# adelacvg/detail_tts

Hardware: AMD Instinct MI355X
Metric: generated audio seconds/sec (24 kHz), 10 s prompt, batch 8 per GPU (higher is better)
Workload: dtype f32; 1 GPU; configs[2]: 1xMI355X batch-8, 10 s prompts (T_ref=936), 234 codes -> 9.984 s audio per utterance; GPT KV-cache decode + 50-step CFG diffusion + flow-VAE/HiFiGAN vocoder, seed-0 random-init weights; batch_per_gpu=8, codes=234, diffusion_steps=50, parallelism=replica x1

## Files before the change

detail_tts_amd/csrc/conv_x3.hip:

```cpp
#include <algorithm>
#include <atomic>
#include <cstdio>
#include <mutex>
#include <type_traits>
#include <utility>
#include <vector>

#include "conv_x3.h"
#include <cstdlib>
#include "prof.h"
#include "split3.h"

namespace dtts {

typedef float f32x16 __attribute__((ext_vector_type(16)));

namespace {
constexpr int NPL = XS_PLANES, NK = 2 * NPL;
constexpr int BM = 128, BN = X3_BN;
constexpr int WTILE = NK * BM * 16;
constexpr int XMAIN = NK * BN * 16;
constexpr int XBUF = XMAIN + NK * 2 * 16;

__global__ __launch_bounds__(256) void split_weights_kernel(const float* __restrict__ wp, int C8, int CoutP, uint4* __restrict__ out) {
// ... 875 lines not shown
    static const long long split_wgs = env_int("DTTS_CONV_KSPLIT_WGS", 256);
    const long long ntile_pad = (long long)(CoutP / BM) * cdiv(Nout, BN) * B;
    static const int max_split_k1 = env_int("DTTS_CONV_KSPLIT_K1", 2);
    if (ntile_pad <= split_tiles) S = (int)std::min<long long>(std::min<long long>(KW == 3 ? max_split : std::min(max_split, max_split_k1), split_wgs / ntile_pad), (Cin >> 4) / 8);
    if (ksplit_max > 0) S = std::min(S, ksplit_max);
    return S < 1 ? 1 : S;
}

static int conv_stages_default() {
    static const int v = []() { const int n = (int)env_int("DTTS_CONV_STAGES", 0); return n >= 2 && n <= 4 ? n : 0; }();
    return v;
}
static std::atomic<int> g_conv_stages{-1};
void set_conv_stages(int n) {
    DTTS_REQUIRE(n <= 0 || (n >= 2 && n <= 4), "conv_stages: 0 (by launch size), 2, 3 or 4");
    g_conv_stages.store(n < 0 ? -1 : n, std::memory_order_relaxed);
}

void launch_conv_x3(const ConvParams& p_in, hipStream_t s, ConvX3Launch* chosen) {
    ConvParams p = p_in;
    DTTS_REQUIRE(p.w3 && p.x3 && (p.y || p.qkv_planes) && p.x3_tp > 0, "conv_x3: operands");
    static const int env_ablate = env_int("DTTS_CONV_ABLATE", 0);
    if (env_ablate) p.ablate = env_ablate;
    DTTS_REQUIRE(p.B > 0 && p.Nout > 0 && p.Cout > 0, "empty conv");
    DTTS_REQUIRE(p.Cin % 16 == 0 && p.CoutP % BM == 0, "conv_x3: channel padding");
    const bool p1 = p.p1 != 0;
    DTTS_REQUIRE(!p1 || (p.Cin % 32 == 0 && p.gate == GATE_NONE), "conv_x3 one-product mode: input channels a multiple of 32, no gate");
    const bool gated = p.gate == GATE_TANH_SIGMOID;
    DTTS_REQUIRE(p.stride == 1 && p.dil == 1 && p.phases == 1 && (p.gate == GATE_NONE ? !p.badd : gated), "conv_x3: unsupported conv form");
    DTTS_REQUIRE(!gated || (p.KW == 1 && !p.qkv_planes && !p.res && p.epi_act == ACT_NONE && p.out_scale == 1.f && p.Cout % 2 == 0),
                 "conv_x3 gated epilogue: 1x1 conv, no residual / activation");
    DTTS_REQUIRE((p.KW == 1 && p.pad == 0) || (p.KW == 3 && p.pad == 1), "conv_x3: k = 1 or k = 3 (same padding) only");
    DTTS_REQUIRE(round_up(p.Nout, BN) + 2 * X3_HALO <= p.x3_tp, "conv_x3: time padding");
    const int stg_opt = g_conv_stages.load(std::memory_order_relaxed);
    const int force_stg = stg_opt >= 0 ? stg_opt : conv_stages_default();
    static const long long max3 = env_int("DTTS_CONV_STAGES3_MAXWG", 600);
    static const long long max4 = env_int("DTTS_CONV_STAGES4_MAXWG", 128);
    DTTS_REQUIRE(!p.cols || (p.ncols > 0 && p.ncols <= cdiv(p.Nout, BN) * p.B && cdiv(p.Nout, BN) < 256), "conv_x3: column table");
    const long long ntile = (long long)(p.CoutP / BM) * (p.cols ? p.ncols : cdiv(p.Nout, BN) * p.B);
    const int S = conv_x3_ksplit(p.CoutP, p.Cin, p.KW, p.Nout, p.B, p.ksplit_max);
    p.ksplit = S;
    static const bool epi_vec_on = env_on("DTTS_X3_EPI_VEC");
    auto al16 = [](const void* q, long long bs, int cs) { return (reinterpret_cast<unsigned long long>(q) & 15ull) == 0 && (bs & 3) == 0 && (cs & 3) == 0; };
    p.epi_vec = (epi_vec_on && p.y && al16(p.y, p.y_bs, p.y_cs) && (!p.res || al16(p.res, p.res_bs, p.res_cs))) ? 1 : 0;
    if (S > 1) {
        const KSplitWs w = ksplit_workspace(s, (size_t)ntile * S);
        p.kpart = w.part;
        p.kcount = w.count;
    }
    const long long nwg = ntile * S;
    static const long long max4k3 = env_int("DTTS_CONV_STAGES4_MAXWG_K3", 128);
    const int nstg = force_stg ? force_stg : (nwg <= (p.KW == 3 ? max4k3 : max4) ? 4 : (nwg <= max3 ? 3 : 2));
    const size_t lds = (size_t)nstg * (WTILE + XBUF) + BM * sizeof(float) + 16;
    const int l4 = 4 * (WTILE + XBUF) + BM * (int)sizeof(float) + 16;
    const dim3 grid((unsigned)nwg);
    const double cols = (double)p.B * p.Nout;
    const double flops = 2.0 * p.Cout * p.Cin * p.KW * cols;
    const double bytes = 4.0 * cols * p.Cin + 4.0 * cols * p.Cout * (p.res ? 2.0 : 1.0) + 4.0 * (double)p.Cout * p.Cin * p.KW;
    {
        static const bool by_shape = []() { const char* v = env_str("DTTS_PROF_SHAPES"); return v && v[0] == '1'; }();
        const char* tag = p1 ? "conv_x3_kernel<128,192,fp16>" : "conv_x3_kernel<128,192>";
        if (by_shape && p1) tag = p.KW == 3 ? "conv_x3 fp16 k3" : (p.Cout > 1024 ? "conv_x3 fp16 k1 M=2304" : (p.res ? "conv_x3 fp16 k1 +res" : "conv_x3 fp16 k1"));
        else if (by_shape) tag = p.KW == 3 ? "conv_x3 k3" : (p.Cout > 1024 ? "conv_x3 k1 M=2304" : (p.res ? "conv_x3 k1 +res" : "conv_x3 k1"));
        ProfScope ps(tag, flops, bytes, s);
        const bool epi = p.epi_act != ACT_NONE || p.out_scale != 1.f;
        if (chosen) {
// ... 48 lines not shown
```

detail_tts_amd/csrc/model.h:

```cpp
#pragma once
#include <map>
#include <memory>
#include <atomic>
#include <thread>
#include <cstring>
#include <memory>
#include <mutex>
#include <string>
#include <unordered_map>
#include <vector>

#include "attention.h"
#include "attn_probs.h"
#include "common.h"
#include "conv_gemm.h"
#include "conv_x3.h"
#include "diff_loss.h"
#include "diff_schedule.h"
#include "disc.h"
#include "flowvae_fwd.h"
#include "gpt_kernels.h"
#include "ops.h"
#include "uncond_cache.h"
#include "../../include/detail_hip.h"

namespace dtts {

struct PackedConv {
    const float* w = nullptr;
    const float* b = nullptr;
    int Cin = 0, CinP = 0, Cout = 0, CoutP = 0, KW = 1;
    const void* w3 = nullptr;
};

static inline int packed_cout(int cout) { return cout > 64 ? round_up(cout, 128) : (cout > 32 ? 64 : 32); }

static inline int gn_groups(int C) {
    int groups = 32;
    while (C % groups) groups /= 2;
    return groups;
}

struct AttnBlockW {
    const float *gn_g = nullptr, *gn_b = nullptr, *bias_tab = nullptr;
    PackedConv qkv, proj;
    int C = 0, H = 0;
};

struct ResBlockW {
    const float *gn1_g = nullptr, *gn1_b = nullptr, *gn2_g = nullptr, *gn2_b = nullptr;
    PackedConv c1, c2, emb;
    int index = 0;
};

struct DiffLayerW {
// ... 305 lines not shown
    void op_attention_x3(const char* name, const float* x, const int* lens_host, int B, int Cin, int T, int H, const float* bias_tab, int p1,
                         int out_f32, void* y, void* img_out, ConvX3Launch* conv_chosen, AttnX3Launch* attn_chosen, hipStream_t s);
    void op_attention(const float* qkv, const int* lens_host, int B, int rows, int cs, int T, int H, int D, int q_off, int k_off, int v_off,
                      int head_stride, float scale, const float* bias_tab, int causal, const float* band, int band_w, float* y, float* ml,
                      hipStream_t s);
    void op_attention_rel(const float* qkv, const int* lens_host, int B, int T, int H, int D, const float* ek, const float* ev, int W,
                          float scale, float* y, float* relk, float* ml, hipStream_t s);
    void op_philox_normal(float* out, int n, int B, unsigned long long seed, const int* sample_ids_host, int stage, int step,
                          hipStream_t s);

    void set_option(const std::string& key, int value) {
        if (key == "two_streams") opt_two_streams_ = value != 0;
        else if (key == "conv_x3") {
            DTTS_REQUIRE(value != 0 || !opt_trunk_fp16_, "conv_x3 = 0 (exact fp32 kernels) has no trunk_fp16 mode: set trunk_fp16 = 0 first");
            opt_conv_x3_ = value != 0;
        }
        else if (key == "trunk_fp16") {
            DTTS_REQUIRE(value == 0 || value == 1, "trunk_fp16: 0 or 1");
            DTTS_REQUIRE(value == 0 || use_x3(), "trunk_fp16 = 1 needs the split-precision kernels (conv_x3 = 1): the exact fp32 kernels have no one-product mode");
            opt_trunk_fp16_ = value != 0;
        }
        else if (key == "gpt_graph") opt_gpt_graph_ = value != 0;
        else if (key == "x3_range_check") opt_range_check_ = value != 0;
        else if (key == "gpt_token_kernel") { opt_gpt_token_ = value != 0; if (value != 0) tok_failed_ = false; gpt_drop_graphs(); }
        else if (key == "gpt_fuse_proj") { DTTS_REQUIRE(value == 0 || value == 1, "gpt_fuse_proj: 0 or 1"); opt_gpt_fuse_proj_ = value != 0; gpt_drop_graphs(); }
        else if (key == "gpt_token_exclusive_cu") { opt_tok_exclusive_ = value != 0; gpt_drop_graphs(); }
        else if (key == "gpt_token_min_rows") { DTTS_REQUIRE(value == 1 || value == 4 || value == 8, "gpt_token_min_rows: 1, 4 or 8"); opt_tok_min_rows_ = value; gpt_drop_graphs(); }
        else if (key == "gpt_token_wgs") { DTTS_REQUIRE(value == 128 || value == 64 || value == 32, "gpt_token_wgs: 128, 64 or 32"); opt_tok_wgs_ = value; gpt_drop_graphs(); }
        else if (key == "gpt_token_fault") opt_tok_fault_ = value;
        else if (key == "gpt_token_fault_eos") opt_tok_fault_eos_ = value;
        else if (key == "gpt_prompt_raw") opt_prompt_raw_ = value != 0;
        else if (key == "gpt_beam_skip_reorder") { opt_beam_skip_reorder_ = value != 0; gpt_drop_graphs(); }
        else if (key == "cfg_streams") opt_cfg_streams_ = value < 0 ? 0 : value;
        else if (key == "conv_cols") opt_conv_cols_ = value != 0;
        else if (key == "uncond_cache_mb") set_uncond_cache_mb(value);
        else if (key == "voc_chain_planes") opt_voc_chain_ = value != 0;
        else if (key == "voc_x3") opt_voc_x3_ = value != 0;
        else if (key == "x3_fault") opt_x3_fault_ = value;
        else if (key == "attn_ksplit_cus") set_attn_ksplit_cus(value);
        else if (key == "attn_ksplit") set_attn_ksplit(value);
        else if (key == "ln_reg") set_ln_channels_reg(value != 0);
        else if (key == "conv_small_tiles") set_conv_small_tiles(value);
        else if (key == "conv_stages") set_conv_stages(value);
        else throw Error(-1, "unknown option '" + key + "'");
    }
    int get_option(const std::string& key) const {
        if (key == "conv_x3") return use_x3() ? 1 : 0;
        if (key == "trunk_fp16") return opt_trunk_fp16_ ? 1 : 0;
        if (key == "gpt_fuse_proj") return opt_gpt_fuse_proj_ ? 1 : 0;
        throw Error(-1, "option '" + key + "' cannot be read back");
    }
    std::string last_error;
    dtts_config cfg;
    int device;

private:
    friend struct Stage;
    const float* W(const std::string& name, size_t numel) const;
    const float* Wopt(const std::string& name, size_t numel) const;
    PackedConv conv(const std::string& name, int Cin, int Cout, int KW, bool bias = true, int cout_p = 0) const;
    AttnBlockW attn_block(const std::string& prefix, int C, int H) const;
    ResBlockW res_block(const std::string& prefix, int C, int index) const;
    void resblock1_fwd(const ResBlock1W& rb, const float* x, float* tmp, float* out, int ch, const int* lens, int B, int T, hipStream_t s,
                       void* xs = nullptr);
    bool vocoder_x3() const;
    void wn_fwd(const WnW& c, float* h, const float* g, int gin, float* Gc, float* acts, float* h2, float* skip, const int* dl, int B,
// ... 37 lines not shown
    void build_vq();
    void build_frontend();
    void gpt_prefill_layers(float* x, const int* lens, int B, int L, float* kv_cache, long long kv_layer_stride, long long kv_bs,
                            int kv_cs, hipStream_t s, const GptAttnCapture* capture = nullptr);
    void gpt_capture_probs(const GptAttnCapture& c, int layer, const float* qkv, const int* lens, int B, int L, hipStream_t s);
    MelStyleW mel_style_w(const std::string& prefix, int n_mel, int hidden, int out) const;
    ConvParams cp(const float* x, int cin, float* y, int cout, int B, int T, int Ta, const int* lens) const;
    ConvParams cp(const float* x, int cin, int Tin, int Tin_a, const int* len_in, float* y, int cout, int Nout, int Nout_a, const int* len_out,
                  int B) const;
    static void with_planes(ConvParams& p, const void* xs, int T) { p.x3 = xs; p.x3_tp = x3_tp(T); }
    static void with_res(ConvParams& p, const float* res, long long bs, int cs) { p.res = res; p.res_bs = bs; p.res_cs = cs; }

    const int* upload_ints(const int* host, int n, hipStream_t s);
    void register_cols(const int* lens_dev, const int* lens_host, int nb, int T, hipStream_t s);

    void run_conv(const PackedConv& pc, ConvParams p, hipStream_t s, ConvX3Launch* chosen = nullptr) const;
    struct TrunkIo {
        const int* lens;
        int B, T, Ta;
        hipStream_t s;
        float* ab;
        void* xs = nullptr;
        bool p1 = false;
        const int* step_idx = nullptr;
    };
    void norm_input(const float* x, int C, const float* gamma, const float* beta, int act, bool x3, const TrunkIo& io);
    void attention_block(const AttnBlockW& w, const float* x, float* y, float* qkv, float* att, const TrunkIo& io);
    void res_block_fwd(const Schedule& sc, const ResBlockW& w, const float* x, float* h1, float* y, int step, const TrunkIo& io);
    void res_block_front(const ResBlockW& w, const float* x, float* h1, const TrunkIo& io);
    void res_block_back(const Schedule& sc, const ResBlockW& w, const float* h1, const float* x, float* y, int step, const TrunkIo& io, int bmod = 0,
                        const int* bidx = nullptr);
    void code_half(const float* in, float* P, const TrunkIo& io);
    bool use_x3() const;
    struct PairPlan { const int *lens2, *lens_i, *umap, *xmap; int Nu; std::vector<int> lens_i_host; };
    PairPlan plan_pair(const int* lens_host, int B, int T, hipStream_t s);
    void diff_forward_pair(const Schedule& sc, const float* x, const float* cbuf0, const PairPlan& pl, int B, int T, int step, float* out2,
                           hipStream_t s, const float* integ = nullptr, const int* umap = nullptr);
    void precompute_integrator(const Schedule& sc, const float* cbuf0, const int* lens_i, const int* lens_i_host, int B, int Nu, int T,
                               const std::vector<int>& steps, float* integ_all, hipStream_t s, int J = 0);
    struct PairCall { PairPlan pl; const int* sids; float *cbuf0, *out2, *hist; bool uncond_deferred; };
    PairCall begin_pair(const float* code_emb, const int* lens_host, const int* sample_ids_host, int B, int T, hipStream_t s,
                        size_t extra_bytes = 0, size_t hist_floats = 0, bool defer_uncond = false);
    void draw_x_T(float* x, const PairCall& pc, const int* lens_host, int B, int T, unsigned long long seed, hipStream_t s);
    struct CodePathTable {
        float* base = nullptr;
        int k0 = 0;
        size_t stride = 0;
        const int* umap = nullptr;
        int umap_stride = 0;
        const float* at(int k) const { return base ? base + (size_t)(k - k0) * stride : nullptr; }
        const int* umap_at(int k) const { return umap ? umap + (size_t)(k - k0) * umap_stride : nullptr; }
    };
    CodePathTable code_path_table(const Schedule& sc, const PairCall& pc, int B, int T, int k_first, int k_end, bool descending, bool pinned,
                                  hipStream_t s);
    enum { SAMPLER_DDIM_REVERSE = 3 };
    void sampler_update(const Schedule& sc, const PairCall& pc, float* x, int B, int T, int sampler, float eta, int step,
                        unsigned long long seed, int pstep, const float* noise, int denorm, hipStream_t s, float* x0_out = nullptr,
                        float* x0_hist = nullptr);
    struct SampleLoop {
        int sampler = 0;
        float eta = 0.f;
        int k_first = 0, k_end = 0;
        int resample = 1;
        const float* known = nullptr;
        const unsigned char* keep = nullptr;
        const float *known_noise = nullptr, *renoise = nullptr;
        const float* step_noise = nullptr;
        float* x_traj = nullptr;
        int denorm = 0;
    };
    void sample_loop(Schedule& sc, const SampleLoop& c, const float* code_emb, const int* lens_host, int B, int T, unsigned long long seed,
                     const int* sample_ids_host, const float* x_init, float* x, hipStream_t s);
    template <class Update>
    void single_step(Schedule& sc, const float* x, const float* code_emb, const int* lens_host, const int* sample_ids_host, int B, int T,
                     int step, bool pinned_table, hipStream_t s, Update&& update);
    void ensure_fork_events();
    void diff_forward_rows_s(const Schedule& sc, const float* x, const float* code_emb, const int* lens_host, int B, int T, const int* step_of_row,
                             float* out, hipStream_t s);
    size_t rows_ws_bytes(int B, int C, int T) const;
    const Schedule& loss_schedule(int sched_id, const int* t_host, int B, const char* who);
    const DiffLossCoefs* upload_loss_coefs(const Schedule& sc, const int* t_host, int B, hipStream_t s);

    std::unordered_map<std::string, std::pair<const float*, size_t>> weights_;
    bool bound_ = false;

    std::vector<DiffLayerW> integ_, layers_;
    std::vector<ResBlockW> tail_;
    std::vector<AttnBlockW> latcond_, ctx_;
    PackedConv xpath_;
    PackedConv integ2_, out_conv_, latcond0_, ctx0_, ctx1_, te0_, te2_;
    const float *out_gn_g_ = nullptr, *out_gn_b_ = nullptr, *code_gn_g_ = nullptr, *code_gn_b_ = nullptr, *uncond_ = nullptr;
    int n_resblocks_ = 0;
    Schedule sched0_;
    static constexpr size_t MAX_SCHEDULES = 8;
    std::vector<std::unique_ptr<Schedule>> sched_cache_;
    int sched_next_id_ = 1;
    std::mutex sched_mu_;
    Schedule& schedule(int id);
    void diff_forward_s(Schedule& sc, const float* x, const float* code_emb, const int* lens_host, int B, int T, int step, int cond_free,
                        float* out, hipStream_t s);
    void build_ss_table(const Schedule& sc, float* ss_table, float* scratch, void* ts_dev, hipStream_t s);
    int cache_schedule(std::unique_ptr<Schedule> key, hipStream_t s);

    MelStyleW ref_enc_, gpt_cond_;
    bool has_vocoder_ = false, has_gpt_ = false;
    PackedConv in_proj_, enc_out_, enc_proj_, dec_pre_, dec_cond_, dec_post_;
    std::vector<EncLayerW> enc_layers_;
    std::vector<CouplingW> flows_;
    PosteriorW enc_q_;
    bool has_enc_q_ = false;
    std::vector<GenStageW> gen_;

// ... 63 lines not shown
    bool ucache_slot_busy(int slot);
    bool integ_unsplit(int Bi_lo, int Bi_hi, int T, int n_pos, int J) const;
public:
    UncondCacheStats uncond_cache_stats();
private:
    int prof_rot_ = 0;
    bool opt_voc_x3_ = true;
    int opt_x3_fault_ = 0;
    bool opt_voc_chain_ = true;
    bool opt_conv_cols_ = true;
    bool opt_range_check_ = false;
    static constexpr int X3_SAT_SLOTS = 8;
    int* x3_sat_ = nullptr;
    int* x3_sat_ring_dev_ = nullptr;
    int* x3_sat_dev_ = nullptr;
    long long x3_ticket_ = 0;
    int* x3_sat_flag(hipStream_t s);
    void x3_sat_check(hipStream_t s);
public:
    long long vocoder_ticket() const { return x3_ticket_; }
    bool vocoder_check_active() const { return x3_sat_dev_ != nullptr && vocoder_x3(); }
    int x3_sat_depth_ = 0;
    struct SatScope {
        Model* m;
        hipStream_t s;
        SatScope(Model* m_, hipStream_t s_) : m(m_), s(s_) { if (m->x3_sat_depth_++ == 0) m->x3_sat_flag(s); }
        ~SatScope() { --m->x3_sat_depth_; }
        void check() { if (m->x3_sat_depth_ == 1) m->x3_sat_check(s); }
        SatScope(const SatScope&) = delete;
        SatScope& operator=(const SatScope&) = delete;
    };
    void vocoder_check(long long ticket);
private:
    int opt_cfg_streams_ = 0;
    bool opt_conv_x3_ = true;
    bool opt_trunk_fp16_ = false;
    Arena w3_;
    Arena w3_voc_;
    static constexpr int MAX_CFG_STREAMS = 4;
    hipStream_t sx_[MAX_CFG_STREAMS - 1] = {nullptr, nullptr, nullptr};
    hipEvent_t ev_fork_ = nullptr, ev_joinx_[MAX_CFG_STREAMS - 1] = {nullptr, nullptr, nullptr};

    bool has_frontend_ = false;
    PackedConv fe_dft_, fe_mel_;
    int fe_nfft_ = 0;

    bool has_vq_ = false;
    MelStyleW vq_ref_enc_;
    PackedConv vq_up1_, vq_up2_, vq_out_;
    const float *vq_table_ = nullptr, *vq_ln_g_ = nullptr, *vq_ln_b_ = nullptr;
    bool has_vq_enc_ = false;
    PackedConv vqe_c1_, vqe_c2_, vqe_c3_, vq_proj_in_;
    const float *vqe_ln_g_ = nullptr, *vqe_ln_b_ = nullptr, *vq_embed_ = nullptr, *vq_embed_sq_ = nullptr;

    Arena ws_main_;
    Arena& ws() { Arena* o = arena_override(); return o ? *o : ws_main_; }
    Arena ws_voc_;
    Arena ws_gpt_;
    Arena persist_;
    struct IntRing {
        static constexpr int SEGS = 16;
        int* dev = nullptr;
        int* pinned = nullptr;
        size_t off = 0;
        int seg = 0;
        std::vector<hipStream_t> users[SEGS];
// ... 13 lines not shown
```

detail_tts_amd/csrc/model_diffusion.hip:

```cpp
#include "model.h"
#include <algorithm>
#include <cmath>
#include <cstring>
#include <optional>
#include "prof.h"

namespace dtts {

static void make_masked_stream(hipStream_t* st, int cus) {
    uint32_t mask[8] = {0, 0, 0, 0, 0, 0, 0, 0};
    for (int b = 0; b < cus; ++b) mask[b >> 5] |= 1u << (b & 31);
    DTTS_CHECK_HIP(hipExtStreamCreateWithCUMask(st, 8, mask));
}

static void make_side_stream(hipStream_t* st) {
    static const int reserve = env_int("DTTS_B_CU_RESERVE", 0);
    if (reserve > 0 && reserve < 256) make_masked_stream(st, 256 - reserve);
    else DTTS_CHECK_HIP(hipStreamCreateWithFlags(st, hipStreamNonBlocking));
}

void Model::ensure_fork_events() {
    if (ev_fork_) return;
    DTTS_CHECK_HIP(hipEventCreateWithFlags(&ev_fork_, hipEventDisableTiming));
    for (auto& e : ev_joinx_) DTTS_CHECK_HIP(hipEventCreateWithFlags(&e, hipEventDisableTiming));
// ... 186 lines not shown
    std::vector<PackedConv*> hot = {&xpath_, &integ2_, &out_conv_};
    auto add_layer = [&](DiffLayerW& l) {
        hot.push_back(&l.rb.c1);
        hot.push_back(&l.rb.c2);
        hot.push_back(&l.at.qkv);
        hot.push_back(&l.at.proj);
    };
    for (auto& l : integ_) add_layer(l);
    for (auto& l : layers_) add_layer(l);
    for (auto& r : tail_) { hot.push_back(&r.c1); hot.push_back(&r.c2); }
    for (auto& b : ctx_) { hot.push_back(&b.qkv); hot.push_back(&b.proj); }
    for (auto& b : latcond_) { hot.push_back(&b.qkv); hot.push_back(&b.proj); }
    size_t total = 0;
    for (PackedConv* pc : hot) {
        DTTS_REQUIRE(pc->Cin == pc->CinP && pc->CoutP % 128 == 0, "trunk conv not eligible for the split-precision path");
        total += (size_t)pc->KW * pc->CinP * pc->CoutP * 4 + 256;
    }
    w3_.ensure(total + 4096);
    for (PackedConv* pc : hot) {
        void* dst = w3_.raw((size_t)pc->KW * pc->CinP * pc->CoutP * 4);
        launch_split_weights(pc->w, pc->KW, pc->CinP, pc->CoutP, dst, s);
        pc->w3 = dst;
    }
}

static size_t qkv_floats(int B, int C, int T) {
    const size_t rows = (size_t)3 * B * C * T, planes = (AttnPlanes::bytes(B, C / AttnPlanes::D, T) + 3) / 4;
    return std::max(rows, planes) + 64;
}

bool Model::use_x3() const {
    static const bool on = env_on("DTTS_CONV_X3");
    return on && opt_conv_x3_;
}

void Model::norm_input(const float* x, int C, const float* gamma, const float* beta, int act, bool x3, const TrunkIo& io) {
    const long long bs = (long long)C * io.Ta;
    if (x3) launch_gn_split_planes(x, bs, io.Ta, io.lens, io.T, io.B, C, gn_groups(C), gamma, beta, 1e-5f, nullptr, 0, 0, act, io.xs, io.s);
    else launch_gn_coeffs(x, bs, io.Ta, io.lens, io.T, io.B, C, gn_groups(C), gamma, beta, 1e-5f, nullptr, 0, 0, io.ab, io.s);
}

void Model::attention_block(const AttnBlockW& w, const float* x, float* y, float* qkv, float* att, const TrunkIo& io) {
    const int C = w.C, D = C / w.H, B = io.B, T = io.T, Ta = io.Ta;
    const long long bs = (long long)C * Ta;
    const bool x3 = io.xs && w.qkv.w3 && w.proj.w3;
    norm_input(x, C, w.gn_g, w.gn_b, ACT_NONE, x3, io);
    ConvParams p = cp(x, C, qkv, 3 * C, B, T, Ta, io.lens);
    p.pro_ab = io.ab;
    const bool planes = x3 && D == AttnPlanes::D;
    DTTS_REQUIRE(!planes || w.bias_tab, "split-precision attention (head dim 48) needs the block's relative-position bias table");
    DTTS_REQUIRE(!io.p1 || planes, "trunk_fp16: the attention has its one-product mode only on the qkv conv's operand images (split-precision path, head dim 48)");
    if (x3) {
        with_planes(p, io.xs, T);
        p.p1 = io.p1;
    }
    if (planes) {
        p.qkv_planes = qkv;
        p.qkv_heads = w.H;
        p.qkv_nt64 = AttnPlanes::nt64(T);
        p.qkv_tq = AttnPlanes::tq(T);
        p.qkv_qscale = (1.f / std::sqrt((float)D)) * 1.4426950408889634f;
    }
    run_conv(w.qkv, p, io.s);
    AttnParams a;
    a.qkv = qkv;
    a.bs = 3 * bs;
    a.cs = Ta;
    a.q_off = 0;
    a.k_off = D;
    a.v_off = 2 * D;
    a.head_stride = 3 * D;
    a.out = att;
    a.o_bs = bs;
    a.o_cs = Ta;
    a.lens = io.lens;
    a.T = T;
    a.B = B;
    a.H = w.H;
    a.D = D;
    a.scale = 1.f / std::sqrt((float)D);
    a.bias_tab = w.bias_tab;
    if (planes) a.planes = qkv;
    a.p1 = io.p1;
    if (RowInvariantLaunches::on()) a.ksplit_max = 1;
    const bool att_planes = planes && T + 1 < x3_tp(T);
    if (att_planes) {
        a.out_x3 = io.xs;
        a.x3_tp = x3_tp(T);
    }
    launch_flash_attention(a, io.s);
    ConvParams q = cp(att, C, y, C, B, T, Ta, io.lens);
    with_res(q, x, bs, Ta);
    if (x3) {
        if (!att_planes) launch_split_planes(att, bs, Ta, nullptr, ACT_NONE, io.lens, T, B, C, io.xs, io.s);
        with_planes(q, io.xs, T);
        q.p1 = io.p1;
    }
    run_conv(w.proj, q, io.s);
}

void Model::res_block_fwd(const Schedule& sc, const ResBlockW& w, const float* x, float* h1, float* y, int step, const TrunkIo& io) {
    res_block_front(w, x, h1, io);
    res_block_back(sc, w, h1, x, y, step, io);
}

void Model::res_block_front(const ResBlockW& w, const float* x, float* h1, const TrunkIo& io) {
    const int C = cfg.diff_channels;
    const bool x3 = io.xs && w.c1.w3 && w.c2.w3;
    norm_input(x, C, w.gn1_g, w.gn1_b, ACT_SILU, x3, io);
    ConvParams p = cp(x, C, h1, C, io.B, io.T, io.Ta, io.lens);
    p.pro_ab = io.ab;
    p.pro_act = ACT_SILU;
    if (x3) {
        with_planes(p, io.xs, io.T);
        p.p1 = io.p1;
    }
    run_conv(w.c1, p, io.s);
}
// ... 41 lines not shown
    pl.lens_i_host = li;
    pl.Nu = (int)ul.size();
    pl.lens2 = upload_ints(l2.data(), 2 * B, s);
    pl.lens_i = upload_ints(li.data(), (int)li.size(), s);
    pl.umap = upload_ints(um.data(), 4 * B, s);
    pl.xmap = pl.umap + 2 * B;
    register_cols(pl.lens2, l2.data(), 2 * B, T, s);
    register_cols(pl.lens_i, li.data(), (int)li.size(), T, s);
    return pl;
}

void Model::diff_forward_pair(const Schedule& sc, const float* x, const float* cbuf0, const PairPlan& pl, int B, int T, int step, float* out2,
                              hipStream_t s, const float* integ, const int* umap) {
    const int C = cfg.diff_channels, Ta = T, OC = cfg.diff_out_channels, MC = cfg.mel_channels, Nu = pl.Nu;
    if (!umap || !integ) umap = pl.umap;
    const int *lens2 = pl.lens2, *lens_i = pl.lens_i;
    const long long bs = (long long)C * Ta;
    static const bool env_two = env_on("DTTS_TWO_STREAMS");
    const bool two_streams = env_two && opt_two_streams_;
    const bool x3 = use_x3();
    DTTS_REQUIRE(!opt_trunk_fp16_ || x3, "trunk_fp16 = 1 needs the split-precision kernels (conv_x3 = 1)");

    void* xs0 = nullptr;
    if (x3) {
        xs0 = ws().raw(x3_bytes(B, MC, T));
        launch_split_planes(x, (long long)MC * T, T, nullptr, ACT_NONE, lens2, T, B, MC, xs0, s);
    }
    static const int env_ns = env_int("DTTS_CFG_STREAMS", 0);
    int NS = env_ns > 0 ? env_ns : (opt_cfg_streams_ > 0 ? opt_cfg_streams_ : (B <= 4 ? 1 : 2));
    if (!two_streams) NS = 1;
    if (NS > MAX_CFG_STREAMS) NS = MAX_CFG_STREAMS;
    while (NS > 1 && ((2 * B) % NS != 0 || (B % ((2 * B) / NS) != 0 && ((2 * B) / NS) % B != 0))) --NS;
    const int n = 2 * B / NS, Bi = B + Nu;
    for (int k = 1; k < NS; ++k)
        if (!sx_[k - 1]) make_side_stream(&sx_[k - 1]);
    if (NS > 1) ensure_fork_events();
    const float* P = integ;
    if (!integ) {
        float* bufP = ws().f32((size_t)Bi * C * Ta);
        const size_t mark = ws().mark();
        const size_t act = (size_t)Bi * C * Ta;
        float* bufI = ws().f32(act);
        float* tA = ws().f32(act);
        float* tB = ws().f32(act);
        float* qkv = ws().f32(qkv_floats(Bi, C, T));
        TrunkIo io{lens_i, Bi, T, Ta, s, ws().f32((size_t)Bi * C * 2)};
        io.xs = x3 ? ws().raw(x3_bytes(Bi, C, T)) : nullptr;
        const float* in = cbuf0;
        for (int l = 0; l < 3; ++l) {
            res_block_fwd(sc, integ_[l].rb, in, tA, tB, step, io);
            attention_block(integ_[l].at, tB, bufI, qkv, tA, io);
            in = bufI;
        }
        code_half(bufI, bufP, io);
        ws().rewind(mark);
        P = bufP;
    }
    if (NS > 1) {
        DTTS_CHECK_HIP(hipEventRecord(ev_fork_, s));
        for (int k = 1; k < NS; ++k) DTTS_CHECK_HIP(hipStreamWaitEvent(sx_[k - 1], ev_fork_, 0));
    }
    for (int k = 0; k < NS; ++k) {
        hipStream_t st = k ? sx_[k - 1] : s;
        const int b0 = k * n;
        const int* lens = lens2 + b0;
        const size_t act = (size_t)n * C * Ta;
        float* bufA = ws().f32(act);
        float* bufB = ws().f32(act);
        float* bufC = ws().f32(act);
        float* qkv = ws().f32(qkv_floats(n, C, T));
        TrunkIo io{lens, n, T, Ta, st, ws().f32((size_t)n * C * 2)};
        io.xs = x3 ? ws().raw(x3_bytes(n, C, T)) : nullptr;
        ConvParams r = cp(x, MC, T, T, lens, bufB, C, T, Ta, lens, n);
        r.pad = 1;
        r.x_bidx = pl.xmap + b0;
        with_res(r, P, bs, Ta);
        r.res_bidx = umap + b0;
        if (x3) with_planes(r, xs0, T);
        run_conv(xpath_, r, st);
        float* cur = bufB;
        float* t1 = bufA;
        float* t2 = bufC;
        for (size_t li = 0; li < layers_.size(); ++li) {
            const auto& l = layers_[li];
            io.p1 = opt_trunk_fp16_ && li >= 1;
            res_block_fwd(sc, l.rb, cur, t1, t2, step, io);
            attention_block(l.at, t2, cur, qkv, t1, io);
        }
        io.p1 = opt_trunk_fp16_;
        for (size_t ti = 0; ti < tail_.size(); ++ti) {
            res_block_fwd(sc, tail_[ti], cur, t1, t2, step, io);
            std::swap(cur, t2);
        }
        norm_input(cur, C, out_gn_g_, out_gn_b_, ACT_SILU, x3, io);
        ConvParams o = cp(cur, C, T, Ta, lens, out2 + (size_t)b0 * OC * T, OC, T, T, lens, n);
        o.pro_ab = io.ab;
        o.pro_act = ACT_SILU;
        o.pad = 1;
        if (x3) with_planes(o, io.xs, T);
        run_conv(out_conv_, o, st);
    }
    for (int k = 1; k < NS; ++k) {
        DTTS_CHECK_HIP(hipEventRecord(ev_joinx_[k - 1], sx_[k - 1]));
        DTTS_CHECK_HIP(hipStreamWaitEvent(s, ev_joinx_[k - 1], 0));
    }
}

void Model::code_half(const float* in, float* P, const TrunkIo& io) {
    const int C = cfg.diff_channels;
    ConvParams r = cp(in, C, P, C, io.B, io.T, io.Ta, io.lens);
    if (io.xs && integ2_.w3) {
        launch_split_planes(in, (long long)C * io.Ta, io.Ta, nullptr, ACT_NONE, io.lens, io.T, io.B, C, io.xs, io.s);
        with_planes(r, io.xs, io.T);
    }
    run_conv(integ2_, r, io.s);
}

size_t Model::rows_ws_bytes(int B, int C, int T) const {
    const size_t act = (size_t)B * C * T;
    return sizeof(float) * (4 * act + qkv_floats(B, C, T) + (size_t)2 * B * C) + x3_bytes(B, cfg.mel_channels, T) + x3_bytes(B, C, T) + 32 * 256;
}

void Model::diff_forward_rows_s(const Schedule& sc, const float* x, const float* code_emb, const int* lens_host, int B, int T,
                                const int* step_of_row, float* out, hipStream_t s) {
    const int C = cfg.diff_channels, Ta = T, OC = cfg.diff_out_channels;
    const long long bs = (long long)C * Ta;
    const size_t act = (size_t)B * C * Ta;
    const bool x3 = use_x3();
    std::vector<int> l(B);
    for (int b = 0; b < B; ++b) l[b] = lens_host ? lens_host[b] : T;
    const int* lens = upload_ints(l.data(), B, s);
    const int* steps = upload_ints(step_of_row, B, s);
    register_cols(lens, l.data(), B, T, s);
    float* bufI = ws().f32(act);
    float* bufA = ws().f32(act);
    float* bufB = ws().f32(act);
    float* bufC = ws().f32(act);
    float* qkv = ws().f32(qkv_floats(B, C, T));
    TrunkIo io{lens, B, T, Ta, s, ws().f32((size_t)B * C * 2)};
    void* xs0 = x3 ? ws().raw(x3_bytes(B, cfg.mel_channels, T)) : nullptr;
    io.xs = x3 ? ws().raw(x3_bytes(B, C, T)) : nullptr;
    io.step_idx = steps;
    const float* in = code_emb;
    for (int li = 0; li < 3; ++li) {
        res_block_fwd(sc, integ_[li].rb, in, bufA, bufB, 0, io);
        attention_block(integ_[li].at, bufB, bufI, qkv, bufA, io);
        in = bufI;
    }
    code_half(bufI, bufC, io);
    ConvParams r = cp(x, cfg.mel_channels, T, T, lens, bufB, C, T, Ta, lens, B);
    r.pad = 1;
    with_res(r, bufC, bs, Ta);
    if (x3) {
        launch_split_planes(x, r.x_bs, T, nullptr, ACT_NONE, lens, T, B, cfg.mel_channels, xs0, s);
        with_planes(r, xs0, T);
    }
    run_conv(xpath_, r, s);
    float* cur = bufB;
    float* t1 = bufA;
    float* t2 = bufC;
    for (const auto& lyr : layers_) {
        res_block_fwd(sc, lyr.rb, cur, t1, t2, 0, io);
        attention_block(lyr.at, t2, cur, qkv, t1, io);
    }
    for (const auto& rb : tail_) {
        res_block_fwd(sc, rb, cur, t1, t2, 0, io);
        std::swap(cur, t2);
    }
    norm_input(cur, C, out_gn_g_, out_gn_b_, ACT_SILU, x3, io);
    ConvParams o = cp(cur, C, T, Ta, lens, out, OC, T, T, lens, B);
    o.pro_ab = io.ab;
    o.pro_act = ACT_SILU;
    o.pad = 1;
    if (x3) with_planes(o, io.xs, T);
    run_conv(out_conv_, o, s);
    if (sc.used) DTTS_CHECK_HIP(hipEventRecord(sc.used, s));
}

void Model::diff_forward_rows(int sched_id, const float* x, const float* code_emb, const int* lens_host, int B, int T, const int* step_of_row,
                              float* out, hipStream_t s) {
    DTTS_REQUIRE(bound_, "weights not bound");
    DTTS_REQUIRE(x && code_emb && step_of_row && out && B >= 1 && T >= 1, "diff_forward_rows: x, code_emb, steps, out");
    DTTS_REQUIRE(!opt_trunk_fp16_, "diff_forward_rows runs the three-product trunk only: set trunk_fp16 = 0 for this call");
    const Schedule& sc = schedule(sched_id);
    DTTS_REQUIRE(sc.kind == 0, "diff_forward_rows runs on an integer-timestep schedule (dtts_diff_schedule)");
    for (int b = 0; b < B; ++b) DTTS_REQUIRE(step_of_row[b] >= 0 && step_of_row[b] < sc.n, "diff_forward_rows: a row's column is outside the schedule");
    ws().ensure(rows_ws_bytes(B, cfg.diff_channels, T) + 8192);
    diff_forward_rows_s(sc, x, code_emb, lens_host, B, T, step_of_row, out, s);
}

static size_t integ_ws_bytes(int Bi, int Bv, int C, int T) {
    const size_t act = (size_t)Bv * C * T;
    return sizeof(float) * ((size_t)Bi * C * T + 2 * (3 * act + qkv_floats(Bv, C, T) + (size_t)2 * Bv * C)) + 2 * x3_bytes(Bv, C, T) + 32 * 256;
}
static int integ_chunk(int Bi) {
    static const int target = env_int("DTTS_INTEG_SAMPLES", 36);
    return std::max(1, target / Bi);
}

void Model::precompute_integrator(const Schedule& sc, const float* cbuf0, const int* lens_i, const int* lens_i_host, int B, int Nu, int T,
                                  const std::vector<int>& steps, float* integ_all, hipStream_t s, int J_call) {
    const int C = cfg.diff_channels, Bi = B + Nu, J = J_call > 0 ? J_call : integ_chunk(Bi), NS = (int)steps.size();
    const size_t ct = (size_t)C * T, mark = ws().mark();
    const int Bv = J * Bi;
    const bool x3 = use_x3();
    static const bool env_two = env_on("DTTS_TWO_STREAMS");
    const bool two = env_two && opt_two_streams_;
    if (two && !sx_[0]) make_side_stream(&sx_[0]);
    hipStream_t side = sx_[0];
    if (two) ensure_fork_events();
    float* h1 = ws().f32((size_t)Bi * ct);
    struct Lane { hipStream_t st; float *bufA, *bufB, *bufC, *qkv, *ab; void* xs; };
    Lane lanes[2];
    for (int q = 0; q < (two ? 2 : 1); ++q) {
        lanes[q].st = q ? side : s;
        lanes[q].bufB = ws().f32((size_t)Bv * ct);
        lanes[q].bufC = ws().f32((size_t)Bv * ct);
        lanes[q].bufA = ws().f32((size_t)Bv * ct);
        lanes[q].qkv = ws().f32(qkv_floats(Bv, C, T));
        lanes[q].ab = ws().f32((size_t)2 * Bv * C);
        lanes[q].xs = x3 ? ws().raw(x3_bytes(Bv, C, T)) : nullptr;
    }
    {
        TrunkIo io0{lens_i, Bi, T, T, s, lanes[0].ab};
        io0.xs = lanes[0].xs;
        res_block_front(integ_[0].rb, cbuf0, h1, io0);
    }
    if (two) {
        DTTS_CHECK_HIP(hipEventRecord(ev_fork_, s));
        DTTS_CHECK_HIP(hipStreamWaitEvent(side, ev_fork_, 0));
    }
    std::vector<int> lv(Bv), sv(Bv), bv(Bv);
    int ci = 0;
    const int prof_rot = prof_rot_++;
    for (int k0 = 0; k0 < NS; k0 += J, ++ci) {
        const Lane& L = lanes[two ? (ci & 1) : 0];
        Profiler::gate() = ((ci / 2 + prof_rot) % Profiler::get().step_every) == 0;
        const int jn = std::min(J, NS - k0), nb = jn * Bi;
        for (int j = 0; j < jn; ++j)
            for (int b = 0; b < Bi; ++b) {
                lv[j * Bi + b] = lens_i_host[b];
                sv[j * Bi + b] = steps[k0 + j];
                bv[j * Bi + b] = b;
            }
        const int* dl = upload_ints(lv.data(), nb, L.st);
        const int* ds = upload_ints(sv.data(), nb, L.st);
        const int* db = x3 ? nullptr : upload_ints(bv.data(), nb, L.st);
        register_cols(dl, lv.data(), nb, T, L.st);
        float* outp = integ_all + (size_t)k0 * Bi * ct;
        TrunkIo io{dl, nb, T, T, L.st, L.ab};
        io.xs = L.xs;
        io.step_idx = ds;
        auto dlayer = [&](const DiffLayerW& l, const float* in, float* o) {
            res_block_fwd(sc, l.rb, in, L.bufB, L.bufC, 0, io);
            attention_block(l.at, L.bufC, o, L.qkv, L.bufB, io);
        };
        res_block_back(sc, integ_[0].rb, h1, cbuf0, L.bufC, 0, io, Bi, db);
        attention_block(integ_[0].at, L.bufC, L.bufA, L.qkv, L.bufB, io);
        dlayer(integ_[1], L.bufA, L.bufA);
        dlayer(integ_[2], L.bufA, L.bufA);
        code_half(L.bufA, outp, io);
        register_cols(dl, nullptr, 0, T, L.st);
    }
    Profiler::gate() = true;
    if (two) {
        DTTS_CHECK_HIP(hipEventRecord(ev_joinx_[0], sx_[0]));
        DTTS_CHECK_HIP(hipStreamWaitEvent(s, ev_joinx_[0], 0));
    }
    ws().rewind(mark);
}

static size_t pair_ws_bytes(int B, int C, int MC, int T) {
    const size_t act = (size_t)B * C * T;
    return sizeof(float) * (2 * act + 2 * (3 * act + qkv_floats(B, C, T) + (size_t)2 * B * C)) + 2 * x3_bytes(B, C, T) + x3_bytes(B, MC, T) + 64 * 256;
}

Model::PairCall Model::begin_pair(const float* code_emb, const int* lens_host, const int* sample_ids_host, int B, int T, hipStream_t s,
                                  size_t extra_bytes, size_t hist_floats, bool defer_uncond) {
    const int C = cfg.diff_channels, OC = cfg.diff_out_channels;
    const size_t half = (size_t)B * C * T;
    ws().ensure(pair_ws_bytes(B, C, cfg.mel_channels, T) + extra_bytes + sizeof(float) * (2 * half + (size_t)2 * B * OC * T + hist_floats) + 8192);
    PairCall pc;
    pc.pl = plan_pair(lens_host, B, T, s);
    pc.sids = sample_ids_host ? upload_ints(sample_ids_host, B, s) : nullptr;
    pc.cbuf0 = ws().f32(2 * half);
    pc.out2 = ws().f32((size_t)2 * B * OC * T);
    pc.hist = hist_floats ? ws().f32(hist_floats) : nullptr;
    if (code_emb) DTTS_CHECK_HIP(hipMemcpyAsync(pc.cbuf0, code_emb, sizeof(float) * half, hipMemcpyDeviceToDevice, s));
    pc.uncond_deferred = defer_uncond;
    for (int h = code_emb ? 1 : 0; h < (defer_uncond ? 1 : 2); ++h)
        launch_broadcast_channels(uncond_, h ? pc.pl.Nu : B, C, T, pc.cbuf0 + h * half, (long long)C * T, T, s);
    return pc;
}

static void check_lens(const int* lens_host, int B, int T) {
    for (int b = 0; lens_host && b < B; ++b) DTTS_REQUIRE(lens_host[b] >= 1 && lens_host[b] <= T, "lens: every length in [1, T]");
}
static bool integ_table_fits(int nst, int B, int C, int T) {
    static const bool env_pre_on = env_on("DTTS_INTEG_PRECOMPUTE");
    static const double max_gb = []() { const char* v = env_str("DTTS_INTEG_MAX_GB"); return v ? atof(v) : 24.0; }();
    return env_pre_on && (double)(sizeof(float) * (size_t)nst * 2 * B * C * T) <= max_gb * 1073741824.0;
}
static size_t integ_call_bytes(int nst, int B, int C, int T) {
    return sizeof(float) * (size_t)nst * 2 * B * C * T + integ_ws_bytes(2 * B, integ_chunk(B + 1) * 2 * B, C, T);
}

void Model::draw_x_T(float* x, const PairCall& pc, const int* lens_host, int B, int T, unsigned long long seed, hipStream_t s) {
    const int MC = cfg.mel_channels;
    const long long xbs = (long long)MC * T;
    DTTS_CHECK_HIP(hipMemsetAsync(x, 0, sizeof(float) * (size_t)B * MC * T, s));
    for (int b = 0; b < B; ++b) {
        const int len = lens_host ? lens_host[b] : T;
        if (len == T) {
            launch_philox_normal(x + (size_t)b * xbs, xbs, MC * T, 1, seed, pc.sids + b, STAGE_DIFF_INIT, 0, 1.f, s);
        } else {
            float* tmp = pc.out2;
            launch_philox_normal(tmp, 0, MC * len, 1, seed, pc.sids + b, STAGE_DIFF_INIT, 0, 1.f, s);
            DTTS_CHECK_HIP(hipMemcpy2DAsync(x + (size_t)b * xbs, sizeof(float) * T, tmp, sizeof(float) * len, sizeof(float) * len, MC,
                                            hipMemcpyDeviceToDevice, s));
        }
    }
}

Model::CodePathTable Model::code_path_table(const Schedule& sc, const PairCall& pc, int B, int T, int k_first, int k_end, bool descending,
                                            bool pinned, hipStream_t s) {
    const PairPlan& pl = pc.pl;
    const int Bi = B + pl.Nu, J = integ_chunk(Bi);
    CodePathTable t;
    t.k0 = pinned ? k_first : k_first / J * J;
    t.stride = (size_t)Bi * cfg.diff_channels * T;
    std::vector<int> steps(k_end - t.k0);
    for (int k = t.k0; k < k_end; ++k) steps[k - t.k0] = descending ? sc.n - 1 - k : k;
    t.base = ws().f32(steps.size() * t.stride);
    std::optional<RowInvariantLaunches> pin;
    if (pinned) pin.emplace();
    const int C = cfg.diff_channels, Nu = pl.Nu, n = (int)steps.size();
    const size_t ct = (size_t)C * T, slab = sizeof(float) * n * ct;
// ... 569 lines not shown
```

Measured before the change: 185.2 audio_s/s.

## Compact diffusion trunk workspace by aliasing activation buffers with qkv scratch

Adds a trunk workspace planner that carves fewer activation buffers for the diffusion trunk. When all convs use split-precision kernels and attention writes planes, h1 aliases the qkv region and y aliases cur, so a residual conv writes in place. The goal is a smaller scratch footprint and better cache locality. The cost is in-place residual writes, which need a new stride guard, plus more complex buffer aliasing that could corrupt data if any kernel reads after another overwrites.

```diff
diff --git a/detail_tts_amd/csrc/conv_x3.hip b/detail_tts_amd/csrc/conv_x3.hip
--- a/detail_tts_amd/csrc/conv_x3.hip
+++ b/detail_tts_amd/csrc/conv_x3.hip
@@ -931,6 +931,8 @@
                  "conv_x3 gated epilogue: 1x1 conv, no residual / activation");
     DTTS_REQUIRE((p.KW == 1 && p.pad == 0) || (p.KW == 3 && p.pad == 1), "conv_x3: k = 1 or k = 3 (same padding) only");
     DTTS_REQUIRE(round_up(p.Nout, BN) + 2 * X3_HALO <= p.x3_tp, "conv_x3: time padding");
+    DTTS_REQUIRE(!p.res || p.res != p.y || (!p.res_bidx && p.res_bmod == 0 && p.res_bs == p.y_bs && p.res_cs == p.y_cs),
+                 "conv_x3: a residual that is the output must have the output's strides and no sample index (res_bidx, res_bmod)");
     const int stg_opt = g_conv_stages.load(std::memory_order_relaxed);
     const int force_stg = stg_opt >= 0 ? stg_opt : conv_stages_default();
     static const long long max3 = env_int("DTTS_CONV_STAGES3_MAXWG", 600);
diff --git a/detail_tts_amd/csrc/model.h b/detail_tts_amd/csrc/model.h
--- a/detail_tts_amd/csrc/model.h
+++ b/detail_tts_amd/csrc/model.h
@@ -21,6 +21,7 @@
 #include "flowvae_fwd.h"
 #include "gpt_kernels.h"
 #include "ops.h"
+#include "trunk_ws.h"
 #include "uncond_cache.h"
 #include "../../include/detail_hip.h"
 
@@ -392,6 +393,7 @@
         else if (key == "gpt_prompt_raw") opt_prompt_raw_ = value != 0;
         else if (key == "gpt_beam_skip_reorder") { opt_beam_skip_reorder_ = value != 0; gpt_drop_graphs(); }
         else if (key == "cfg_streams") opt_cfg_streams_ = value < 0 ? 0 : value;
+        else if (key == "trunk_compact_ws") { DTTS_REQUIRE(value == 0 || value == 1, "trunk_compact_ws: 0 or 1"); opt_trunk_compact_ = value != 0; }
         else if (key == "conv_cols") opt_conv_cols_ = value != 0;
         else if (key == "uncond_cache_mb") set_uncond_cache_mb(value);
         else if (key == "voc_chain_planes") opt_voc_chain_ = value != 0;
@@ -495,6 +497,8 @@
                         const int* bidx = nullptr);
     void code_half(const float* in, float* P, const TrunkIo& io);
     bool use_x3() const;
+    TrunkPlan trunk_plan(int T) const;
+    TrunkShape trunk_shape(int T) const;
     struct PairPlan { const int *lens2, *lens_i, *umap, *xmap; int Nu; std::vector<int> lens_i_host; };
     PairPlan plan_pair(const int* lens_host, int B, int T, hipStream_t s);
     void diff_forward_pair(const Schedule& sc, const float* x, const float* cbuf0, const PairPlan& pl, int B, int T, int step, float* out2,
@@ -541,6 +545,7 @@
     void diff_forward_rows_s(const Schedule& sc, const float* x, const float* code_emb, const int* lens_host, int B, int T, const int* step_of_row,
                              float* out, hipStream_t s);
     size_t rows_ws_bytes(int B, int C, int T) const;
+    size_t integ_call_bytes(int nst, int B, int C, int T) const;
     const Schedule& loss_schedule(int sched_id, const int* t_host, int B, const char* who);
     const DiffLossCoefs* upload_loss_coefs(const Schedule& sc, const int* t_host, int B, hipStream_t s);
 
@@ -670,6 +675,7 @@
     };
     void vocoder_check(long long ticket);
 private:
+    bool opt_trunk_compact_ = true;
     int opt_cfg_streams_ = 0;
     bool opt_conv_x3_ = true;
     bool opt_trunk_fp16_ = false;
diff --git a/detail_tts_amd/csrc/model_diffusion.hip b/detail_tts_amd/csrc/model_diffusion.hip
--- a/detail_tts_amd/csrc/model_diffusion.hip
+++ b/detail_tts_amd/csrc/model_diffusion.hip
@@ -242,6 +242,35 @@
 bool Model::use_x3() const {
     static const bool on = env_on("DTTS_CONV_X3");
     return on && opt_conv_x3_;
+}
+
+static bool attn_writes_planes(const AttnBlockW& w, bool x3, int T) {
+    return x3 && w.qkv.w3 && w.proj.w3 && w.C / w.H == AttnPlanes::D && T + 1 < x3_tp(T);
+}
+
+TrunkPlan Model::trunk_plan(int T) const {
+    if (!opt_trunk_compact_ || !use_x3()) return TRUNK_3BUF;
+    bool planes = true;
+    auto block = [&](const ResBlockW& rb) { return rb.c1.w3 && rb.c2.w3; };
+    auto layer = [&](const DiffLayerW& l) {
+        if (!attn_writes_planes(l.at, true, T)) planes = false;
+        return block(l.rb) && l.at.qkv.w3 && l.at.proj.w3;
+    };
+    for (const auto& l : integ_) if (!layer(l)) return TRUNK_3BUF;
+    for (const auto& l : layers_) if (!layer(l)) return TRUNK_3BUF;
+    for (const auto& r : tail_) if (!block(r)) return TRUNK_3BUF;
+    if (!xpath_.w3 || !integ2_.w3) return TRUNK_3BUF;
+    return planes ? TRUNK_COMPACT : TRUNK_OWN_H1;
+}
+
+TrunkShape Model::trunk_shape(int T) const {
+    TrunkShape sh;
+    sh.C = cfg.diff_channels;
+    sh.T = T;
+    sh.qkv1 = qkv_floats(1, sh.C, T) - 64;
+    sh.xs1 = use_x3() ? x3_bytes(1, sh.C, T) : 0;
+    DTTS_REQUIRE(sh.dims(3).qkv == qkv_floats(3, sh.C, T) && sh.dims(3).qkv >= sh.dims(3).act, "trunk_shape: the qkv region is per-sample and holds h1");
+    return sh;
 }
 
 void Model::norm_input(const float* x, int C, const float* gamma, const float* beta, int act, bool x3, const TrunkIo& io) {
@@ -293,7 +322,7 @@
     if (planes) a.planes = qkv;
     a.p1 = io.p1;
     if (RowInvariantLaunches::on()) a.ksplit_max = 1;
-    const bool att_planes = planes && T + 1 < x3_tp(T);
+    const bool att_planes = planes && attn_writes_planes(w, x3, T);
     if (att_planes) {
         a.out_x3 = io.xs;
         a.x3_tp = x3_tp(T);
@@ -401,6 +430,8 @@
     if (NS > MAX_CFG_STREAMS) NS = MAX_CFG_STREAMS;
     while (NS > 1 && ((2 * B) % NS != 0 || (B % ((2 * B) / NS) != 0 && ((2 * B) / NS) % B != 0))) --NS;
     const int n = 2 * B / NS, Bi = B + Nu;
+    const TrunkPlan plan = trunk_plan(T);
+    const TrunkShape shape = trunk_shape(T);
     for (int k = 1; k < NS; ++k)
         if (!sx_[k - 1]) make_side_stream(&sx_[k - 1]);
     if (NS > 1) ensure_fork_events();
@@ -408,20 +439,16 @@
     if (!integ) {
         float* bufP = ws().f32((size_t)Bi * C * Ta);
         const size_t mark = ws().mark();
-        const size_t act = (size_t)Bi * C * Ta;
-        float* bufI = ws().f32(act);
-        float* tA = ws().f32(act);
-        float* tB = ws().f32(act);
-        float* qkv = ws().f32(qkv_floats(Bi, C, T));
-        TrunkIo io{lens_i, Bi, T, Ta, s, ws().f32((size_t)Bi * C * 2)};
-        io.xs = x3 ? ws().raw(x3_bytes(Bi, C, T)) : nullptr;
+        const TrunkScratch t = carve_trunk(ws(), shape.dims(Bi), plan);
+        TrunkIo io{lens_i, Bi, T, Ta, s, t.ab};
+        io.xs = t.xs;
         const float* in = cbuf0;
         for (int l = 0; l < 3; ++l) {
-            res_block_fwd(sc, integ_[l].rb, in, tA, tB, step, io);
-            attention_block(integ_[l].at, tB, bufI, qkv, tA, io);
-            in = bufI;
+            res_block_fwd(sc, integ_[l].rb, in, t.h1, t.y, step, io);
+            attention_block(integ_[l].at, t.y, t.cur, t.qkv, t.h1, io);
+            in = t.cur;
         }
-        code_half(bufI, bufP, io);
+        code_half(t.cur, bufP, io);
         ws().rewind(mark);
         P = bufP;
     }
@@ -433,23 +460,20 @@
         hipStream_t st = k ? sx_[k - 1] : s;
         const int b0 = k * n;
         const int* lens = lens2 + b0;
-        const size_t act = (size_t)n * C * Ta;
-        float* bufA = ws().f32(act);
-        float* bufB = ws().f32(act);
-        float* bufC = ws().f32(act);
-        float* qkv = ws().f32(qkv_floats(n, C, T));
-        TrunkIo io{lens, n, T, Ta, st, ws().f32((size_t)n * C * 2)};
-        io.xs = x3 ? ws().raw(x3_bytes(n, C, T)) : nullptr;
-        ConvParams r = cp(x, MC, T, T, lens, bufB, C, T, Ta, lens, n);
+        const TrunkScratch t = carve_trunk(ws(), shape.dims(n), plan);
+        float* const qkv = t.qkv;
+        TrunkIo io{lens, n, T, Ta, st, t.ab};
+        io.xs = t.xs;
+        ConvParams r = cp(x, MC, T, T, lens, t.cur, C, T, Ta, lens, n);
         r.pad = 1;
         r.x_bidx = pl.xmap + b0;
         with_res(r, P, bs, Ta);
         r.res_bidx = umap + b0;
         if (x3) with_planes(r, xs0, T);
         run_conv(xpath_, r, st);
-        float* cur = bufB;
-        float* t1 = bufA;
-        float* t2 = bufC;
+        float* cur = t.cur;
+        float* t1 = t.h1;
+        float* t2 = t.y;
         for (size_t li = 0; li < layers_.size(); ++li) {
             const auto& l = layers_[li];
             io.p1 = opt_trunk_fp16_ && li >= 1;
@@ -486,8 +510,8 @@
 }
 
 size_t Model::rows_ws_bytes(int B, int C, int T) const {
-    const size_t act = (size_t)B * C * T;
-    return sizeof(float) * (4 * act + qkv_floats(B, C, T) + (size_t)2 * B * C) + x3_bytes(B, cfg.mel_channels, T) + x3_bytes(B, C, T) + 32 * 256;
+    DTTS_REQUIRE(C == cfg.diff_channels, "rows_ws_bytes: the trunk's channels");
+    return trunk_rows_ws_bytes(trunk_shape(T), B, trunk_plan(T), x3_bytes(B, cfg.mel_channels, T));
 }
 
 void Model::diff_forward_rows_s(const Schedule& sc, const float* x, const float* code_emb, const int* lens_host, int B, int T,
@@ -502,32 +526,31 @@
     const int* steps = upload_ints(step_of_row, B, s);
     register_cols(lens, l.data(), B, T, s);
     float* bufI = ws().f32(act);
-    float* bufA = ws().f32(act);
-    float* bufB = ws().f32(act);
-    float* bufC = ws().f32(act);
-    float* qkv = ws().f32(qkv_floats(B, C, T));
-    TrunkIo io{lens, B, T, Ta, s, ws().f32((size_t)B * C * 2)};
+    const TrunkScratch t = carve_trunk(ws(), trunk_shape(T).dims(B), trunk_plan(T));
+    float* const qkv = t.qkv;
+    TrunkIo io{lens, B, T, Ta, s, t.ab};
     void* xs0 = x3 ? ws().raw(x3_bytes(B, cfg.mel_channels, T)) : nullptr;
-    io.xs = x3 ? ws().raw(x3_bytes(B, C, T)) : nullptr;
+    io.xs = t.xs;
     io.step_idx = steps;
     const float* in = code_emb;
     for (int li = 0; li < 3; ++li) {
-        res_block_fwd(sc, integ_[li].rb, in, bufA, bufB, 0, io);
-        attention_block(integ_[li].at, bufB, bufI, qkv, bufA, io);
+        float* yI = t.y == t.cur ? bufI : t.y;
+        res_block_fwd(sc, integ_[li].rb, in, t.h1, yI, 0, io);
+        attention_block(integ_[li].at, yI, bufI, qkv, t.h1, io);
         in = bufI;
     }
-    code_half(bufI, bufC, io);
-    ConvParams r = cp(x, cfg.mel_channels, T, T, lens, bufB, C, T, Ta, lens, B);
+    code_half(bufI, t.y, io);
+    ConvParams r = cp(x, cfg.mel_channels, T, T, lens, t.cur, C, T, Ta, lens, B);
     r.pad = 1;
-    with_res(r, bufC, bs, Ta);
+    with_res(r, t.y, bs, Ta);
     if (x3) {
         launch_split_planes(x, r.x_bs, T, nullptr, ACT_NONE, lens, T, B, cfg.mel_channels, xs0, s);
         with_planes(r, xs0, T);
     }
     run_conv(xpath_, r, s);
-    float* cur = bufB;
-    float* t1 = bufA;
-    float* t2 = bufC;
+    float* cur = t.cur;
+    float* t1 = t.h1;
+    float* t2 = t.y;
     for (const auto& lyr : layers_) {
         res_block_fwd(sc, lyr.rb, cur, t1, t2, 0, io);
         attention_block(lyr.at, t2, cur, qkv, t1, io);
@@ -558,10 +581,6 @@
     diff_forward_rows_s(sc, x, code_emb, lens_host, B, T, step_of_row, out, s);
 }
 
-static size_t integ_ws_bytes(int Bi, int Bv, int C, int T) {
-    const size_t act = (size_t)Bv * C * T;
-    return sizeof(float) * ((size_t)Bi * C * T + 2 * (3 * act + qkv_floats(Bv, C, T) + (size_t)2 * Bv * C)) + 2 * x3_bytes(Bv, C, T) + 32 * 256;
-}
 static int integ_chunk(int Bi) {
     static const int target = env_int("DTTS_INTEG_SAMPLES", 36);
     return std::max(1, target / Bi);
@@ -579,20 +598,17 @@
     hipStream_t side = sx_[0];
     if (two) ensure_fork_events();
     float* h1 = ws().f32((size_t)Bi * ct);
-    struct Lane { hipStream_t st; float *bufA, *bufB, *bufC, *qkv, *ab; void* xs; };
+    struct Lane { hipStream_t st; TrunkScratch t; };
     Lane lanes[2];
+    const TrunkPlan plan = trunk_plan(T);
+    const TrunkDims dims = trunk_shape(T).dims(Bv);
     for (int q = 0; q < (two ? 2 : 1); ++q) {
         lanes[q].st = q ? side : s;
-        lanes[q].bufB = ws().f32((size_t)Bv * ct);
-        lanes[q].bufC = ws().f32((size_t)Bv * ct);
-        lanes[q].bufA = ws().f32((size_t)Bv * ct);
-        lanes[q].qkv = ws().f32(qkv_floats(Bv, C, T));
-        lanes[q].ab = ws().f32((size_t)2 * Bv * C);
-        lanes[q].xs = x3 ? ws().raw(x3_bytes(Bv, C, T)) : nullptr;
+        lanes[q].t = carve_trunk(ws(), dims, plan);
     }
     {
-        TrunkIo io0{lens_i, Bi, T, T, s, lanes[0].ab};
-        io0.xs = lanes[0].xs;
+        TrunkIo io0{lens_i, Bi, T, T, s, lanes[0].t.ab};
+        io0.xs = lanes[0].t.xs;
         res_block_front(integ_[0].rb, cbuf0, h1, io0);
     }
     if (two) {
@@ -617,18 +633,19 @@
         const int* db = x3 ? nullptr : upload_ints(bv.data(), nb, L.st);
         register_cols(dl, lv.data(), nb, T, L.st);
         float* outp = integ_all + (size_t)k0 * Bi * ct;
-        TrunkIo io{dl, nb, T, T, L.st, L.ab};
-        io.xs = L.xs;
+        const TrunkScratch& t = L.t;
+        TrunkIo io{dl, nb, T, T, L.st, t.ab};
+        io.xs = t.xs;
         io.step_idx = ds;
-        auto dlayer = [&](const DiffLayerW& l, const float* in, float* o) {
-            res_block_fwd(sc, l.rb, in, L.bufB, L.bufC, 0, io);
-            attention_block(l.at, L.bufC, o, L.qkv, L.bufB, io);
+        auto dlayer = [&](const DiffLayerW& l) {
+            res_block_fwd(sc, l.rb, t.cur, t.h1, t.y, 0, io);
+            attention_block(l.at, t.y, t.cur, t.qkv, t.h1, io);
         };
-        res_block_back(sc, integ_[0].rb, h1, cbuf0, L.bufC, 0, io, Bi, db);
-        attention_block(integ_[0].at, L.bufC, L.bufA, L.qkv, L.bufB, io);
-        dlayer(integ_[1], L.bufA, L.bufA);
-        dlayer(integ_[2], L.bufA, L.bufA);
-        code_half(L.bufA, outp, io);
+        res_block_back(sc, integ_[0].rb, h1, cbuf0, t.y, 0, io, Bi, db);
+        attention_block(integ_[0].at, t.y, t.cur, t.qkv, t.h1, io);
+        dlayer(integ_[1]);
+        dlayer(integ_[2]);
+        code_half(t.cur, outp, io);
         register_cols(dl, nullptr, 0, T, L.st);
     }
     Profiler::gate() = true;
@@ -639,16 +656,11 @@
     ws().rewind(mark);
 }
 
-static size_t pair_ws_bytes(int B, int C, int MC, int T) {
-    const size_t act = (size_t)B * C * T;
-    return sizeof(float) * (2 * act + 2 * (3 * act + qkv_floats(B, C, T) + (size_t)2 * B * C)) + 2 * x3_bytes(B, C, T) + x3_bytes(B, MC, T) + 64 * 256;
-}
-
 Model::PairCall Model::begin_pair(const float* code_emb, const int* lens_host, const int* sample_ids_host, int B, int T, hipStream_t s,
                                   size_t extra_bytes, size_t hist_floats, bool defer_uncond) {
     const int C = cfg.diff_channels, OC = cfg.diff_out_channels;
     const size_t half = (size_t)B * C * T;
-    ws().ensure(pair_ws_bytes(B, C, cfg.mel_channels, T) + extra_bytes + sizeof(float) * (2 * half + (size_t)2 * B * OC * T + hist_floats) + 8192);
+    ws().ensure(trunk_pair_ws_bytes(trunk_shape(T), B, trunk_plan(T), x3_bytes(B, cfg.mel_channels, T)) + extra_bytes + sizeof(float) * (2 * half + (size_t)2 * B * OC * T + hist_floats) + 8192);
     PairCall pc;
     pc.pl = plan_pair(lens_host, B, T, s);
     pc.sids = sample_ids_host ? upload_ints(sample_ids_host, B, s) : nullptr;
@@ -670,8 +682,8 @@
     static const double max_gb = []() { const char* v = env_str("DTTS_INTEG_MAX_GB"); return v ? atof(v) : 24.0; }();
     return env_pre_on && (double)(sizeof(float) * (size_t)nst * 2 * B * C * T) <= max_gb * 1073741824.0;
 }
-static size_t integ_call_bytes(int nst, int B, int C, int T) {
-    return sizeof(float) * (size_t)nst * 2 * B * C * T + integ_ws_bytes(2 * B, integ_chunk(B + 1) * 2 * B, C, T);
+size_t Model::integ_call_bytes(int nst, int B, int C, int T) const {
+    return sizeof(float) * (size_t)nst * 2 * B * C * T + trunk_integ_ws_bytes(trunk_shape(T), 2 * B, integ_chunk(B + 1) * 2 * B, trunk_plan(T));
 }
 
 void Model::draw_x_T(float* x, const PairCall& pc, const int* lens_host, int B, int T, unsigned long long seed, hipStream_t s) {
diff --git a/detail_tts_amd/csrc/trunk_ws.h b/detail_tts_amd/csrc/trunk_ws.h
--- /dev/null
+++ b/detail_tts_amd/csrc/trunk_ws.h
@@ -0,0 +1,62 @@
+#pragma once
+#include <cstddef>
+
+namespace dtts {
+
+enum TrunkPlan { TRUNK_COMPACT = 1, TRUNK_OWN_H1 = 2, TRUNK_3BUF = 3 };
+
+struct TrunkDims {
+    size_t act = 0;
+    size_t qkv = 0;
+    size_t ab = 0;
+    size_t xs = 0;
+};
+
+struct TrunkShape {
+    int C = 0, T = 0;
+    size_t qkv1 = 0, xs1 = 0;
+    TrunkDims dims(int n) const {
+        TrunkDims d;
+        d.act = (size_t)n * C * T;
+        d.qkv = (size_t)n * qkv1 + 64;
+        d.ab = (size_t)2 * n * C;
+        d.xs = (size_t)n * xs1;
+        return d;
+    }
+};
+
+struct TrunkScratch {
+    float *cur = nullptr, *h1 = nullptr, *y = nullptr, *qkv = nullptr, *ab = nullptr;
+    void* xs = nullptr;
+};
+
+template <class A>
+TrunkScratch carve_trunk(A& ws, const TrunkDims& d, TrunkPlan plan) {
+    auto f32 = [&](size_t n) { return static_cast<float*>(ws.raw(n * sizeof(float))); };
+    TrunkScratch t;
+    if (plan != TRUNK_COMPACT) t.h1 = f32(d.act);
+    t.cur = f32(d.act);
+    t.y = plan == TRUNK_3BUF ? f32(d.act) : t.cur;
+    t.qkv = f32(d.qkv);
+    if (plan == TRUNK_COMPACT) t.h1 = t.qkv;
+    t.ab = f32(d.ab);
+    t.xs = d.xs ? ws.raw(d.xs) : nullptr;
+    return t;
+}
+
+static inline size_t trunk_stack_bytes(const TrunkDims& d, TrunkPlan plan) {
+    return sizeof(float) * ((size_t)plan * d.act + d.qkv + d.ab) + d.xs;
+}
+static_assert(TRUNK_COMPACT == 1 && TRUNK_OWN_H1 == 2 && TRUNK_3BUF == 3, "the enumerator counts the plan's activation buffers");
+
+static inline size_t trunk_pair_ws_bytes(const TrunkShape& sh, int B, TrunkPlan plan, size_t xs0) {
+    return sizeof(float) * 2 * sh.dims(B).act + 2 * trunk_stack_bytes(sh.dims(B), plan) + xs0 + 64 * 256;
+}
+static inline size_t trunk_integ_ws_bytes(const TrunkShape& sh, int Bi, int Bv, TrunkPlan plan) {
+    return sizeof(float) * sh.dims(Bi).act + 2 * trunk_stack_bytes(sh.dims(Bv), plan) + 32 * 256;
+}
+static inline size_t trunk_rows_ws_bytes(const TrunkShape& sh, int B, TrunkPlan plan, size_t xs0) {
+    return sizeof(float) * sh.dims(B).act + trunk_stack_bytes(sh.dims(B), plan) + xs0 + 32 * 256;
+}
+
+}
```

Measured after the change: 186.9 audio_s/s (median of 6 runs). No clear change (+0.9%).
